# bryanlimy/tf2-cyclegan

Measured on AMD Instinct MI355X. Metric: images/sec (whole node) horse2zebra 256×256, higher is better.
Workload: dtype bf16; 1 GPU; model=cyclegan-resnet9-patchgan, global_batch=4, per_gpu_batch=4, image_size=256, parallelism=dp1

## Files before the change

cyclegan_amd/ops/_hip/bind.cpp:

```cpp
#include <torch/extension.h>

namespace cyg {
at::Tensor conv2d_fwd(at::Tensor, at::Tensor, c10::optional<at::Tensor>,
                      int64_t, int64_t, int64_t, int64_t, int64_t, bool,
                      int64_t, double);
at::Tensor convt2d_fwd(at::Tensor, at::Tensor, c10::optional<at::Tensor>,
                       int64_t, int64_t, int64_t, int64_t, int64_t, int64_t,
                       double);
std::vector<at::Tensor> conv2d_fwd_stats(at::Tensor, at::Tensor,
                                         c10::optional<at::Tensor>, int64_t,
                                         int64_t, int64_t, int64_t, int64_t,
                                         bool, int64_t, double);
std::vector<at::Tensor> convt2d_fwd_stats(at::Tensor, at::Tensor,
                                          c10::optional<at::Tensor>, int64_t,
                                          int64_t, int64_t, int64_t, int64_t,
                                          int64_t, double);
at::Tensor conv2d_dgrad(at::Tensor, at::Tensor, int64_t, int64_t, int64_t,
                        int64_t, int64_t, int64_t, int64_t, bool);
at::Tensor reflect_dgrad_rowmap(int64_t, int64_t, int64_t, int64_t, int64_t,
                                int64_t, int64_t, int64_t, int64_t, bool,
                                bool);
at::Tensor convt2d_dgrad(at::Tensor, at::Tensor, int64_t, int64_t, int64_t,
                         int64_t, int64_t);
at::Tensor conv2d_wgrad(at::Tensor, at::Tensor, int64_t, int64_t, int64_t,
// ... 23 lines not shown
                                     c10::optional<at::Tensor>, int64_t);
std::vector<at::Tensor> instnorm_fwd_q8(at::Tensor, at::Tensor, at::Tensor,
                                        double, int64_t, double,
                                        c10::optional<at::Tensor>,
                                        c10::optional<at::Tensor>,
                                        c10::optional<at::Tensor>, int64_t,
                                        at::Tensor, at::Tensor);
std::vector<at::Tensor> instnorm_bwd(at::Tensor, at::Tensor, at::Tensor,
                                     at::Tensor, at::Tensor,
                                     c10::optional<at::Tensor>, int64_t,
                                     double, c10::optional<at::Tensor>,
                                     c10::optional<at::Tensor>,
                                     c10::optional<at::Tensor>, bool);
at::Tensor act_bwd(at::Tensor, at::Tensor, int64_t, double);
at::Tensor channel_sum(at::Tensor, c10::optional<at::Tensor>, bool);
at::Tensor reflect_pad_fwd(at::Tensor, int64_t, int64_t, int64_t, int64_t);
at::Tensor reflect_pad_bwd(at::Tensor, int64_t, int64_t, int64_t, int64_t);
at::Tensor persample_loss_fwd(at::Tensor, at::Tensor, bool);
at::Tensor persample_loss_const_fwd(at::Tensor, double, bool);
std::vector<at::Tensor> persample_loss_bwd(at::Tensor, at::Tensor, at::Tensor,
                                           bool, bool, bool);
at::Tensor persample_loss_const_bwd(at::Tensor, double, at::Tensor, bool);
void adam_step_dev(at::Tensor, at::Tensor, at::Tensor, at::Tensor, at::Tensor,
                   double, double, double);
void adam_ema_step(at::Tensor, at::Tensor, at::Tensor, at::Tensor, at::Tensor,
                   double, double, double, double, int64_t, double);
void adam_ema_step_dev(at::Tensor, at::Tensor, at::Tensor, at::Tensor,
                       at::Tensor, at::Tensor, double, double, double, double);
void shadow_gather(at::Tensor, at::Tensor, at::Tensor);
void shadow_fold(at::Tensor, at::Tensor, at::Tensor);
void fold_upconv_dw_into(at::Tensor, at::Tensor, bool, bool);
void adam_step(at::Tensor, at::Tensor, at::Tensor, at::Tensor, double, double,
               double, double, int64_t);
at::Tensor augment_batch(at::Tensor, at::Tensor, at::Tensor, int64_t, int64_t,
                         at::Tensor);
at::Tensor pool_exchange(at::Tensor, at::Tensor, at::Tensor, at::Tensor);
std::vector<at::Tensor> ssim_fwd(at::Tensor, at::Tensor, int64_t);
at::Tensor ssim_bwd(at::Tensor, at::Tensor, at::Tensor, at::Tensor, at::Tensor,
                    at::Tensor);
}

PYBIND11_MODULE(TORCH_EXTENSION_NAME, m) {
  m.def("conv2d_fwd", &cyg::conv2d_fwd);
  m.def("convt2d_fwd", &cyg::convt2d_fwd);
  m.def("conv2d_fwd_stats", &cyg::conv2d_fwd_stats);
  m.def("convt2d_fwd_stats", &cyg::convt2d_fwd_stats);
  m.def("conv2d_dgrad", &cyg::conv2d_dgrad);
  m.def("reflect_dgrad_rowmap", &cyg::reflect_dgrad_rowmap, py::arg("B"),
        py::arg("H"), py::arg("W"), py::arg("pt"), py::arg("pb"),
        py::arg("pl"), py::arg("pr"), py::arg("KH"), py::arg("KW"),
        py::arg("trim") = true, py::arg("frame") = false);
  m.def("convt2d_dgrad", &cyg::convt2d_dgrad);
  m.def("conv2d_wgrad", &cyg::conv2d_wgrad);
  m.def("conv2d_wgrad_into", &cyg::conv2d_wgrad_into, py::arg("x"),
        py::arg("dy"), py::arg("kh"), py::arg("kw"), py::arg("stride"),
        py::arg("pt"), py::arg("pl"), py::arg("reflect"), py::arg("out"),
// ... 13 lines not shown
  m.def("instnorm_fwd", &cyg::instnorm_fwd, py::arg("x"), py::arg("gamma"),
        py::arg("beta"), py::arg("eps"), py::arg("act"), py::arg("slope"),
        py::arg("residual"), py::arg("psum") = py::none(),
        py::arg("psq") = py::none(), py::arg("nslabs") = 0);
  m.def("instnorm_fwd_q8", &cyg::instnorm_fwd_q8, py::arg("x"),
        py::arg("gamma"), py::arg("beta"), py::arg("eps"), py::arg("act"),
        py::arg("slope"), py::arg("residual"), py::arg("psum"),
        py::arg("psq"), py::arg("nslabs"), py::arg("amax_prev"),
        py::arg("amax_cur"));
  m.def("instnorm_bwd", &cyg::instnorm_bwd, py::arg("dy"), py::arg("x"),
        py::arg("gamma"), py::arg("mean"), py::arg("rstd"), py::arg("yact"),
        py::arg("act"), py::arg("slope"), py::arg("beta") = py::none(),
        py::arg("dgamma_out") = py::none(), py::arg("dbeta_out") = py::none(),
        py::arg("accumulate") = false);
  m.def("act_bwd", &cyg::act_bwd);
  m.def("channel_sum", &cyg::channel_sum, py::arg("x"),
        py::arg("out") = py::none(), py::arg("accumulate") = false);
  m.def("reflect_pad_fwd", &cyg::reflect_pad_fwd);
  m.def("reflect_pad_bwd", &cyg::reflect_pad_bwd);
  m.def("persample_loss_fwd", &cyg::persample_loss_fwd);
  m.def("persample_loss_const_fwd", &cyg::persample_loss_const_fwd);
  m.def("persample_loss_bwd", &cyg::persample_loss_bwd);
  m.def("persample_loss_const_bwd", &cyg::persample_loss_const_bwd);
  m.def("adam_step", &cyg::adam_step);
  m.def("adam_step_dev", &cyg::adam_step_dev);
  m.def("adam_ema_step", &cyg::adam_ema_step);
  m.def("adam_ema_step_dev", &cyg::adam_ema_step_dev);
  m.def("shadow_gather", &cyg::shadow_gather);
  m.def("shadow_fold", &cyg::shadow_fold);
  m.def("fold_upconv_dw_into", &cyg::fold_upconv_dw_into, py::arg("dv"),
        py::arg("out"), py::arg("accumulate"), py::arg("transposed"));
  m.def("augment_batch", &cyg::augment_batch);
  m.def("pool_exchange", &cyg::pool_exchange);
  m.def("ssim_fwd", &cyg::ssim_fwd, py::arg("y_true"), py::arg("y_pred"),
        py::arg("save_maps") = 0);
  m.def("ssim_bwd", &cyg::ssim_bwd, py::arg("x"), py::arg("y"), py::arg("am"),
        py::arg("bm"), py::arg("cm"), py::arg("dout"));
}
```

cyclegan_amd/ops/_hip/common.h:

```cpp
#pragma once

#include <hip/hip_runtime.h>
#include <hip/hip_bf16.h>
#include <hip/hip_fp8.h>

#define DEV __device__ __forceinline__

typedef __bf16 bf16r;
typedef bf16r v8bf __attribute__((ext_vector_type(8)));
typedef float v4f __attribute__((ext_vector_type(4)));
typedef short v8s __attribute__((ext_vector_type(8)));

DEV float b2f(short raw) {
  union { float f; unsigned u; } v;
  v.u = ((unsigned)(unsigned short)raw) << 16;
  return v.f;
}

DEV short f2b(float f) {
  __hip_bfloat16 h = __float2bfloat16(f);
  return *reinterpret_cast<short*>(&h);
}

DEV float delayed_sx(float amax_prev) {
  return fminf(448.f / fmaxf(amax_prev, 1e-12f), 65504.f);
}

DEV unsigned char f2e4m3(float f, float s) {
  __hip_fp8_e4m3 q(f * s);
  return q.__x;
}

#define ACT_NONE 0
#define ACT_RELU 1
// ... 23 lines not shown
```

cyclegan_amd/ops/_hip/norm_elem.hip:

```cpp

#include <torch/extension.h>
#include <ATen/cuda/CUDAContext.h>

#include "common.h"

namespace cyg {

constexpr int NT = 256;

static inline int cdiv64(long a, long b) { return (int)((a + b - 1) / b); }

__global__ __launch_bounds__(NT) void in_reduce_kernel(
    const short* __restrict__ x, float* __restrict__ psum,
    float* __restrict__ psq, int B, long HW, int C, int S) {
  int b = blockIdx.x / S;
  int sl = blockIdx.x % S;
  long rows = (HW + S - 1) / S;
  long r0 = sl * rows, r1 = min(r0 + rows, HW);
  const int gpr = C / 8;
  const int tid = threadIdx.x;
  const short* xb = x + (long)b * HW * C;

  int g = tid % gpr;
  int rstep = NT / gpr;
// ... 564 lines not shown
  if (i >= D) return;
  float t = use_const ? cconst : b2f(yt[base + i]);
  float p = b2f(yp[base + i]);
  float d = p - t;
  float g = dout[b] / (float)D;
  float gpv = squared ? 2.f * d * g : (d > 0.f ? g : (d < 0.f ? -g : 0.f));
  if (gp) gp[base + i] = f2b(gpv);
  if (gt) gt[base + i] = f2b(-gpv);
  (void)n;
}

__device__ __forceinline__ void adam_elem(float& p, float g, float& m,
                                          float& v, float lr_t, float b1,
                                          float b2, float eps) {
#pragma clang fp contract(off)
  float gi = g;
  float mi = b1 * m + (1.f - b1) * gi;
  float vi = b2 * v + (1.f - b2) * gi * gi;
  m = mi;
  v = vi;
  p -= lr_t * mi / (sqrtf(vi) + eps);
}

__global__ void adam_kernel(float* __restrict__ p, const float* __restrict__ g,
                            float* __restrict__ m, float* __restrict__ v,
                            long n, float lr_t, float b1, float b2,
                            float eps) {
  long i = (long)blockIdx.x * blockDim.x + threadIdx.x;
  long stride = (long)gridDim.x * blockDim.x;
  for (; i < n; i += stride)
    adam_elem(p[i], g[i], m[i], v[i], lr_t, b1, b2, eps);
}

__global__ void adam_kernel_dev(float* __restrict__ p,
                                const float* __restrict__ g,
                                float* __restrict__ m, float* __restrict__ v,
                                long n, const float* __restrict__ lr_t_ptr,
                                float b1, float b2, float eps) {
  const float lr_t = *lr_t_ptr;
  long i = (long)blockIdx.x * blockDim.x + threadIdx.x;
  long stride = (long)gridDim.x * blockDim.x;
  for (; i < n; i += stride)
    adam_elem(p[i], g[i], m[i], v[i], lr_t, b1, b2, eps);
}

__device__ __forceinline__ void adam_ema_elem(float& p, float g, float& m,
                                              float& v, float& e, float lr_t,
                                              float b1, float b2, float eps,
                                              float d, float omd) {
#pragma clang fp contract(off)
  adam_elem(p, g, m, v, lr_t, b1, b2, eps);
  e = d * e + omd * p;
}

template <bool VEC, bool LR_DEV>
__global__ void adam_ema_kernel(float* __restrict__ p,
                                const float* __restrict__ g,
                                float* __restrict__ m, float* __restrict__ v,
                                float* __restrict__ ema, long n, float lr_imm,
                                const float* __restrict__ lr_t_ptr, float b1,
                                float b2, float eps, float d, float omd) {
  const float lr_t = LR_DEV ? *lr_t_ptr : lr_imm;
  const long tid = (long)blockIdx.x * blockDim.x + threadIdx.x;
  const long stride = (long)gridDim.x * blockDim.x;
  long done = 0;
  if (VEC) {
    const long n4 = n >> 2;
    float4* p4 = reinterpret_cast<float4*>(p);
    const float4* g4 = reinterpret_cast<const float4*>(g);
    float4* m4 = reinterpret_cast<float4*>(m);
    float4* v4 = reinterpret_cast<float4*>(v);
    float4* e4 = reinterpret_cast<float4*>(ema);
    for (long i = tid; i < n4; i += stride) {
      float4 pi = p4[i], gi = g4[i], mi = m4[i], vi = v4[i], ei = e4[i];
      adam_ema_elem(pi.x, gi.x, mi.x, vi.x, ei.x, lr_t, b1, b2, eps, d, omd);
      adam_ema_elem(pi.y, gi.y, mi.y, vi.y, ei.y, lr_t, b1, b2, eps, d, omd);
      adam_ema_elem(pi.z, gi.z, mi.z, vi.z, ei.z, lr_t, b1, b2, eps, d, omd);
      adam_ema_elem(pi.w, gi.w, mi.w, vi.w, ei.w, lr_t, b1, b2, eps, d, omd);
      m4[i] = mi;
      v4[i] = vi;
      p4[i] = pi;
      e4[i] = ei;
    }
    done = n4 << 2;
  }
  for (long i = done + tid; i < n; i += stride)
    adam_ema_elem(p[i], g[i], m[i], v[i], ema[i], lr_t, b1, b2, eps, d, omd);
}


static int slices_for(long HW, int B) {
  int s = (int)std::min<long>(std::max<long>(1, 512 / std::max(B, 1)),
                              std::max<long>(1, HW / 64));
  return std::max(1, s);
}

static std::vector<at::Tensor> instnorm_fwd_impl(
    at::Tensor x, at::Tensor gamma, at::Tensor beta, double eps, int64_t act,
    double slope, c10::optional<at::Tensor> residual,
    c10::optional<at::Tensor> psum_in, c10::optional<at::Tensor> psq_in,
    int64_t nslabs, const at::Tensor* amax_prev, at::Tensor* amax_cur) {
  TORCH_CHECK(x.is_cuda() && x.scalar_type() == at::kBFloat16 && x.is_contiguous());
  int B = x.size(0), C = x.size(3);
  long HW = (long)x.size(1) * x.size(2);
  TORCH_CHECK(C % 8 == 0 && (C / 8) <= 256 && 256 % std::min(C / 8, 256) == 0,
              "instnorm: unsupported channel count ", C);
  auto stream = at::cuda::getCurrentCUDAStream();
  auto fopt = x.options().dtype(at::kFloat);
  int S = slices_for(HW, B);
  auto mean = at::empty({B, C}, fopt);
// ... 320 lines not shown
                     (const short*)yp.const_data_ptr(),
                     (const float*)dout.const_data_ptr(),
                     need_gt ? (short*)gt.mutable_data_ptr() : nullptr,
                     need_gp ? (short*)gp.mutable_data_ptr() : nullptr, D,
                     squared ? 1 : 0, 0.f, 0);
  return {gt, gp};
}

at::Tensor persample_loss_const_bwd(at::Tensor yp, double cconst,
                                    at::Tensor dout, bool squared) {
  int B = yp.size(0);
  long D = yp.numel() / B;
  auto gp = at::empty_like(yp);
  dim3 grid(cdiv64(D, 256), B);
  hipLaunchKernelGGL(persample_loss_bwd_kernel, grid, dim3(256), 0,
                     at::cuda::getCurrentCUDAStream(), nullptr,
                     (const short*)yp.const_data_ptr(),
                     (const float*)dout.const_data_ptr(), nullptr,
                     (short*)gp.mutable_data_ptr(), D, squared ? 1 : 0,
                     (float)cconst, 1);
  return gp;
}

void adam_step(at::Tensor p, at::Tensor g, at::Tensor m, at::Tensor v,
               double lr, double b1, double b2, double eps, int64_t t) {
  TORCH_CHECK(p.is_cuda() && p.scalar_type() == at::kFloat);
  long n = p.numel();
  double lr_t = lr * std::sqrt(1.0 - std::pow(b2, (double)t)) /
                (1.0 - std::pow(b1, (double)t));
  int blocks = (int)std::min<long>(2048, (n + 255) / 256);
  hipLaunchKernelGGL(adam_kernel, dim3(blocks), dim3(256), 0,
                     at::cuda::getCurrentCUDAStream(),
                     (float*)p.mutable_data_ptr(),
                     (const float*)g.const_data_ptr(),
                     (float*)m.mutable_data_ptr(),
                     (float*)v.mutable_data_ptr(), n, (float)lr_t, (float)b1,
                     (float)b2, (float)eps);
}

void adam_step_dev(at::Tensor p, at::Tensor g, at::Tensor m, at::Tensor v,
                   at::Tensor lr_t, double b1, double b2, double eps) {
  TORCH_CHECK(p.is_cuda() && p.scalar_type() == at::kFloat);
  TORCH_CHECK(lr_t.is_cuda() && lr_t.scalar_type() == at::kFloat);
  long n = p.numel();
  int blocks = (int)std::min<long>(2048, (n + 255) / 256);
  hipLaunchKernelGGL(adam_kernel_dev, dim3(blocks), dim3(256), 0,
                     at::cuda::getCurrentCUDAStream(),
                     (float*)p.mutable_data_ptr(),
                     (const float*)g.const_data_ptr(),
                     (float*)m.mutable_data_ptr(),
                     (float*)v.mutable_data_ptr(), n,
                     (const float*)lr_t.const_data_ptr(), (float)b1,
                     (float)b2, (float)eps);
}

static void adam_ema_launch(at::Tensor& p, at::Tensor& g, at::Tensor& m,
                            at::Tensor& v, at::Tensor& ema, float lr_imm,
                            const float* lr_t_ptr, double b1, double b2,
                            double eps, double ema_decay) {
  TORCH_CHECK(p.is_cuda() && p.scalar_type() == at::kFloat);
  for (const at::Tensor* t : {&p, &g, &m, &v, &ema}) {
    TORCH_CHECK(t->scalar_type() == at::kFloat, "adam_ema: fp32 only");
    TORCH_CHECK(t->numel() == p.numel(), "adam_ema: numel mismatch");
    TORCH_CHECK(t->is_contiguous(), "adam_ema: contiguous only");
    TORCH_CHECK(t->device() == p.device(), "adam_ema: device mismatch");
  }
  TORCH_CHECK(ema_decay >= 0.0 && ema_decay <= 1.0);
  long n = p.numel();
  if (n == 0) return;
  float* pp = (float*)p.mutable_data_ptr();
  const float* gp = (const float*)g.const_data_ptr();
  float* mp = (float*)m.mutable_data_ptr();
  float* vp = (float*)v.mutable_data_ptr();
  float* ep = (float*)ema.mutable_data_ptr();
  bool vec = ((reinterpret_cast<uintptr_t>(pp) |
               reinterpret_cast<uintptr_t>(gp) |
               reinterpret_cast<uintptr_t>(mp) |
               reinterpret_cast<uintptr_t>(vp) |
               reinterpret_cast<uintptr_t>(ep)) & 15) == 0;
  float d = (float)ema_decay, omd = (float)(1.0 - ema_decay);
  long work = vec ? std::max<long>(n >> 2, n & 3) : n;
  int blocks = (int)std::min<long>(2048, (work + 255) / 256);
  auto stream = at::cuda::getCurrentCUDAStream();
#define CYG_ADAM_EMA(VEC, LRD)                                              \
  hipLaunchKernelGGL((adam_ema_kernel<VEC, LRD>), dim3(blocks), dim3(256),  \
                     0, stream, pp, gp, mp, vp, ep, n, lr_imm, lr_t_ptr,    \
                     (float)b1, (float)b2, (float)eps, d, omd)
  if (lr_t_ptr) {
    if (vec) CYG_ADAM_EMA(true, true); else CYG_ADAM_EMA(false, true);
  } else {
    if (vec) CYG_ADAM_EMA(true, false); else CYG_ADAM_EMA(false, false);
  }
#undef CYG_ADAM_EMA
}

void adam_ema_step(at::Tensor p, at::Tensor g, at::Tensor m, at::Tensor v,
                   at::Tensor ema, double lr, double b1, double b2,
                   double eps, int64_t t, double ema_decay) {
  double lr_t = lr * std::sqrt(1.0 - std::pow(b2, (double)t)) /
                (1.0 - std::pow(b1, (double)t));
  adam_ema_launch(p, g, m, v, ema, (float)lr_t, nullptr, b1, b2, eps,
                  ema_decay);
}

void adam_ema_step_dev(at::Tensor p, at::Tensor g, at::Tensor m, at::Tensor v,
                       at::Tensor ema, at::Tensor lr_t, double b1, double b2,
                       double eps, double ema_decay) {
  TORCH_CHECK(lr_t.is_cuda() && lr_t.scalar_type() == at::kFloat &&
              lr_t.numel() == 1 && lr_t.device() == p.device());
  adam_ema_launch(p, g, m, v, ema, 0.f, (const float*)lr_t.const_data_ptr(),
                  b1, b2, eps, ema_decay);
}

}
```

cyclegan_amd/ops/_hip/shadow.hip:

```cpp

#include <torch/extension.h>
#include <ATen/cuda/CUDAContext.h>

#include "common.h"

namespace cyg {

constexpr int SG_NT = 256;

typedef int v8i __attribute__((ext_vector_type(8)));

__global__ __launch_bounds__(SG_NT) void shadow_gather_kernel(
    const float* __restrict__ src, const int* __restrict__ idx,
    short* __restrict__ out, long n8) {
  long t = (long)blockIdx.x * SG_NT + threadIdx.x;
  long stride = (long)gridDim.x * SG_NT;
  for (; t < n8; t += stride) {
    v8i ix = *(const v8i*)(idx + t * 8);
    v8s o;
    #pragma unroll
    for (int j = 0; j < 8; ++j)
      o[j] = ix[j] >= 0 ? f2b(src[ix[j]]) : (short)0;
    *(v8s*)(out + t * 8) = o;
  }
}

void shadow_gather(at::Tensor src, at::Tensor idx, at::Tensor out) {
  TORCH_CHECK(src.is_cuda() && src.scalar_type() == at::kFloat &&
              src.is_contiguous());
  TORCH_CHECK(idx.is_cuda() && idx.scalar_type() == at::kInt &&
              idx.is_contiguous());
  TORCH_CHECK(out.is_cuda() && out.scalar_type() == at::kBFloat16 &&
              out.is_contiguous());
  TORCH_CHECK(idx.numel() == out.numel() && idx.numel() % 8 == 0);
  long n8 = idx.numel() / 8;
  int blocks = (int)min((long)4096, (n8 + SG_NT - 1) / SG_NT);
  hipLaunchKernelGGL(shadow_gather_kernel, dim3(blocks), dim3(SG_NT), 0,
                     at::cuda::getCurrentCUDAStream(),
                     (const float*)src.const_data_ptr(),
                     (const int*)idx.const_data_ptr(),
                     (short*)out.mutable_data_ptr(), n8);
}

typedef int v4i __attribute__((ext_vector_type(4)));

__global__ __launch_bounds__(SG_NT) void shadow_fold_kernel(
    const float* __restrict__ src, const int* __restrict__ idx4,
    short* __restrict__ out, long n8) {
  long t = (long)blockIdx.x * SG_NT + threadIdx.x;
  long stride = (long)gridDim.x * SG_NT;
  for (; t < n8; t += stride) {
    v8s o;
    #pragma unroll
    for (int j = 0; j < 8; ++j) {
      v4i ix = *(const v4i*)(idx4 + (t * 8 + j) * 4);
      float s = 0.f;
      #pragma unroll
      for (int q = 0; q < 4; ++q)
        if (ix[q] >= 0) s += src[ix[q]];
      o[j] = f2b(s);
    }
    *(v8s*)(out + t * 8) = o;
  }
}
// ... 68 lines not shown
```

cyclegan_amd/ops/adam.py:

```python

from __future__ import annotations

import math

import torch

from . import backend


class FusedAdam:

    def __init__(self, flat_param: torch.Tensor, flat_grad: torch.Tensor,
                 lr: float = 2e-4, beta1: float = 0.5, beta2: float = 0.9,
                 eps: float = 1e-7, ema_decay: float = 0.0):
        assert flat_param.dtype == torch.float32
        assert 0.0 <= ema_decay < 1.0
        self.p = flat_param
        self.g = flat_grad
        self.lr, self.b1, self.b2, self.eps = lr, beta1, beta2, eps
        self.m = torch.zeros_like(flat_param)
        self.v = torch.zeros_like(flat_param)
        self.t = 0
        self.lr_scale = 1.0
        self.ema_decay = float(ema_decay)
        self.ema = flat_param.detach().clone() if ema_decay > 0 else None
        self.graph_mode = False
        self._lr_t_dev = None

    def _lr_t(self) -> float:
        return (self.lr * self.lr_scale * math.sqrt(1 - self.b2 ** self.t)
                / (1 - self.b1 ** self.t))

    @torch.no_grad()
    def reset_ema(self):
        if self.ema is not None:
            self.ema.copy_(self.p)

    @torch.no_grad()
    def prepare_graph(self):
        self.graph_mode = True
        if self._lr_t_dev is None:
            self._lr_t_dev = torch.zeros(1, dtype=torch.float32,
                                         device=self.p.device)

    @torch.no_grad()
    def advance_lr(self):
        self.t += 1
        if self._lr_t_dev is None:
            self._lr_t_dev = torch.empty(1, dtype=torch.float32,
                                         device=self.p.device)
        self._lr_t_dev.fill_(self._lr_t())

    @torch.no_grad()
    def step(self):
        if self.graph_mode:
            if self.ema is not None:
                backend.ext().adam_ema_step_dev(
                    self.p, self.g, self.m, self.v, self.ema, self._lr_t_dev,
                    self.b1, self.b2, self.eps, self.ema_decay)
                return
            backend.ext().adam_step_dev(self.p, self.g, self.m, self.v,
                                        self._lr_t_dev, self.b1, self.b2,
                                        self.eps)
            return
        self.t += 1
        if backend.use_hip(self.p):
            lr = self.lr * self.lr_scale
            if self.ema is not None:
                backend.ext().adam_ema_step(
                    self.p, self.g, self.m, self.v, self.ema, lr, self.b1,
                    self.b2, self.eps, self.t, self.ema_decay)
            else:
                backend.ext().adam_step(self.p, self.g, self.m, self.v,
                                        lr, self.b1, self.b2, self.eps, self.t)
            torch.autograd.graph.increment_version(self.p)
            return
        lr_t = (self.lr * self.lr_scale * math.sqrt(1 - self.b2 ** self.t)
                / (1 - self.b1 ** self.t))
        self.m.mul_(self.b1).add_(self.g, alpha=1 - self.b1)
        self.v.mul_(self.b2).addcmul_(self.g, self.g, value=1 - self.b2)
        self.p.addcdiv_(self.m, self.v.sqrt().add_(self.eps), value=-lr_t)
        if self.ema is not None:
            self.ema.mul_(self.ema_decay).add_(self.p, alpha=1 - self.ema_decay)

    def state_dict(self):
        return {"m": self.m, "v": self.v, "t": self.t,
                "lr": self.lr, "b1": self.b1, "b2": self.b2, "eps": self.eps}

    def load_state_dict(self, sd):
        self.m.copy_(sd["m"])
        self.v.copy_(sd["v"])
        self.t = sd["t"]
        self.lr, self.b1, self.b2, self.eps = sd["lr"], sd["b1"], sd["b2"], sd["eps"]
```

cyclegan_amd/ops/arena.py:

```python

from __future__ import annotations

from typing import Dict, List, Tuple

import torch

from . import backend

_PAD = 8


def _conv_like(m: torch.nn.Module) -> bool:
    return type(m).__name__ == "ConvNHWC"


def _convt_like(m: torch.nn.Module) -> bool:
    return type(m).__name__ == "ConvTransposeNHWC"


def _upconv_like(m: torch.nn.Module) -> bool:
    return type(m).__name__ == "UpsampleConvNHWC"


FOLD_M = ((0, 0, 1), (0, 1, 1), (1, 1, 0), (1, 0, 0))
_FOLD_TAPS = tuple(tuple(d for d in range(3) if row[d]) for row in FOLD_M)


def _idx_up(base: int, shape) -> torch.Tensor:
    O, KH, KW, I = shape
    assert KH == 3 and KW == 3
    o = torch.arange(O).view(-1, 1)
    i = torch.arange(I).view(1, -1)
# ... 54 lines not shown
    assert KW == 7
    d = torch.arange(8).view(-1, 1, 1, 1, 1, 1)
    co = torch.arange(8).view(1, -1, 1, 1, 1, 1)
    ty = torch.arange(KH).view(1, 1, -1, 1, 1, 1)
    blk = torch.arange(2).view(1, 1, 1, -1, 1, 1)
    pos = torch.arange(8).view(1, 1, 1, 1, -1, 1)
    ci = torch.arange(I).view(1, 1, 1, 1, 1, -1)
    tx = blk * 8 + pos - d
    idx = base + ((co * KH + ty) * KW + tx) * I + ci
    ok = (tx >= 0) & (tx < KW) & (co < O)
    idx = torch.where(ok, idx, torch.tensor(-1))
    return idx.reshape(64, KH, 2, 8 * I).to(torch.int32)


def _idx_packb(base: int, n: int) -> torch.Tensor:
    co = torch.arange(8).repeat(8)
    idx = base + co
    idx[co >= n] = -1
    return idx.to(torch.int32)


class ShadowArena:

    def __init__(self, group, module: torch.nn.Module):
        self.group = group
        dev = group.flat_param.device
        off = {p: o for p, (o, _) in zip(group.params, group._offsets)}

        pieces: List[torch.Tensor] = []
        plan: List[Tuple[torch.nn.Parameter, str, Tuple[int, ...], int]] = []
        total = 0
        fpieces: List[torch.Tensor] = []
        fplan: List[Tuple[torch.nn.Parameter, str, Tuple[int, ...], int]] = []
        ftotal = 0
        for m in module.modules():
            if _upconv_like(m):
                w = m.weight
                for name, fn in (("up", _idx_up), ("up_t", _idx_up_t)):
                    idx = fn(off[w], tuple(w.shape))
                    fpieces.append(idx.reshape(-1, 4))
                    fplan.append((w, name, tuple(idx.shape[:-1]), ftotal))
                    ftotal += idx.numel() // 4
                continue
            if _conv_like(m):
                forms = (("p", _idx_p), ("tp", _idx_tp))
            elif _convt_like(m):
                forms = (("plain", _idx_plain), ("t", _idx_t))
            else:
                continue
            w = m.weight
            forms = list(forms)
            packed = (_conv_like(m) and head_packable(
                tuple(w.shape), m.stride, m.pad_mode, m.padding
                if not isinstance(m.padding, str) else (0,) * 4))
            if packed:
                forms.append(("packp", _idx_packp))
            for name, fn in forms:
                idx = fn(off[w], tuple(w.shape))
                pieces.append(idx.reshape(-1))
                plan.append((w, name, tuple(idx.shape), total))
                total += idx.numel()
            if m.bias is not None:
                idx = _idx_bias(off[m.bias], m.bias.numel())
                pieces.append(idx.reshape(-1))
                plan.append((m.bias, "bias_p", tuple(idx.shape), total))
                total += idx.numel()
                if packed:
                    idx = _idx_packb(off[m.bias], m.bias.numel())
                    pieces.append(idx.reshape(-1))
                    plan.append((m.bias, "packb", tuple(idx.shape), total))
                    total += idx.numel()

        pad = (-total) % 8
        if pad:
            pieces.append(torch.full((pad,), -1, dtype=torch.int32))
        self.idx = torch.cat(pieces).to(dev) if pieces else \
            torch.empty(0, dtype=torch.int32, device=dev)
        self.buf = torch.empty(self.idx.numel(), dtype=torch.bfloat16, device=dev)

        fpad = (-ftotal) % 8
        if fpad:
            fpieces.append(torch.full((fpad, 4), -1, dtype=torch.int32))
        self.fold_idx = torch.cat(fpieces).to(dev) if fpieces else \
            torch.empty((0, 4), dtype=torch.int32, device=dev)
        self.fold_buf = torch.empty(self.fold_idx.shape[0],
                                    dtype=torch.bfloat16, device=dev)

        self.views: Dict[Tuple[int, str], torch.Tensor] = {}
        self._by_param: Dict[torch.Tensor, Dict[str, torch.Tensor]] = {}
        for p, name, shape, start in plan:
            v = self.buf[start:start + int(torch.tensor(shape).prod())].view(shape)
            self._by_param.setdefault(p, {})[name] = v
        for p, name, shape, start in fplan:
            v = self.fold_buf[start:start + int(torch.tensor(shape).prod())]
            self._by_param.setdefault(p, {})[name] = v.view(shape)

        self.refresh()

    def refresh(self):
        if self.idx.numel():
            backend.ext().shadow_gather(self.group.flat_param, self.idx, self.buf)
        if self.fold_idx.numel():
            backend.ext().shadow_fold(self.group.flat_param, self.fold_idx,
                                      self.fold_buf)

    def forms_of(self, p: torch.Tensor):
        return self._by_param.get(p)
```

cyclegan_amd/trainer.py:

```python

from __future__ import annotations

import contextlib
import os
from typing import Dict, Optional

import torch

from .models import Generator, Discriminator
from .ops import MAE, MSE, MSE_const, SSIM, ImagePool, backend, grad_sink
from .ops.adam import FusedAdam
from .parallel import DistContext, GradSync, FlatParamGroup


def lr_factor(epoch: int, epochs: int, decay_epochs: int) -> float:
    if decay_epochs <= 0:
        return 1.0
    f = 1.0 - max(0, epoch - (epochs - decay_epochs) + 1) / (decay_epochs + 1)
    return min(1.0, max(0.0, f))


class CycleGAN:
    LAMBDA_CYCLE = 10.0
    LAMBDA_IDENTITY = 0.5 * 10.0
# ... 28 lines not shown
        for m in (self.G, self.F, self.X, self.Y):
            ctx.broadcast_module(m)

        self.groups = {name: FlatParamGroup(getattr(self, name))
                       for name in self._NAMES}
        self.ema_decay = float(getattr(args, "ema_decay", 0.0) or 0.0)
        self.lr_decay_epochs = int(getattr(args, "lr_decay_epochs", 0) or 0)
        self.optimizers = {
            name: FusedAdam(g.flat_param, g.flat_grad,
                            ema_decay=self.ema_decay if name in "GF" else 0.0)
            for name, g in self.groups.items()}
        self.sync = GradSync(ctx, timing=getattr(args, "verbose", 1) == 2)

        self.arenas = {}
        if (self.device.type == "cuda"
                and self.compute_dtype == torch.bfloat16
                and backend.load_ext() is not None):
            from .ops.arena import ShadowArena
            from .ops import shadow as _shadow
            for name in self._NAMES:
                a = ShadowArena(self.groups[name], getattr(self, name))
                _shadow.register_arena(a)
                self.arenas[name] = a

        self.pool_size = int(getattr(args, "pool_size", 0) or 0)
        self._pool_seed = (int(getattr(args, "seed", 1234)), int(ctx.rank))
        self.pools = None
        self._step_codes = None
        self._static_codes = None

        self.cycle_ssim = float(getattr(args, "cycle_ssim", 0.0) or 0.0)
        if not 0.0 <= self.cycle_ssim <= 1.0:
            raise ValueError("cycle_ssim must be in [0, 1]")
        self.test_ssim = (bool(getattr(args, "test_ssim", False))
                          or self.cycle_ssim > 0.0)
        self._test_keys = self._TEST_KEYS + (
            self._SSIM_KEYS if self.test_ssim else ())

        self.graphed = None

    def _refresh_shadows(self):
        for a in self.arenas.values():
            a.refresh()

    def _snapshot_state(self):
        opts = self.optimizers
        return ({n: (g.flat_param.clone(), opts[n].m.clone(),
                     opts[n].v.clone(), opts[n].t)
                 for n, g in self.groups.items()},
                {n: o.ema.clone() for n, o in opts.items()
                 if o.ema is not None},
                [p.state_dict() for p in self.pools or ()])

    @torch.no_grad()
    def _restore_state(self, saved):
        state, emas, pools = saved
        for n, (p, m, v, t) in state.items():
            self.groups[n].flat_param.copy_(p)
            self.optimizers[n].m.copy_(m)
            self.optimizers[n].v.copy_(v)
            self.optimizers[n].t = t
        for n, e in emas.items():
            self.optimizers[n].ema.copy_(e)
        for p, s in zip(self.pools or (), pools):
            p.load_state_dict(s)
        self._refresh_shadows()
# ... 174 lines not shown

    _GROUP_LOSS = tuple(zip(_NAMES, ("loss_G/total", "loss_F/total",
                                     "loss_X/loss", "loss_Y/loss")))

    def _grads_for(self, losses: Dict[str, torch.Tensor], name: str,
                   retain: bool):
        key = dict(self._GROUP_LOSS)[name]
        group = self.groups[name]
        sink = group.grad_sink()
        with grad_sink.active(sink):
            grads = torch.autograd.grad(losses[key], group.params,
                                        retain_graph=retain,
                                        allow_unused=sink is not None)
        group.set_grads(grads, sink)

    def _retain(self, i: int) -> bool:
        return i < 3 and not self.pool_size

    def _optimize(self, roll_amax: bool = True):
        for opt in self.optimizers.values():
            opt.step()
        for g in self.groups.values():
            g.bump_versions()
        self._refresh_shadows()
        if self._fp8 and roll_amax:
            from .ops import fp8_state
            fp8_state.roll()

    def train_step(self, x, y) -> Dict[str, torch.Tensor]:
        x, y = self._cast(x), self._cast(y)
        if x.shape[0] == 0:
            return self._empty_train_step()
        if self.pool_size:
            self._step_codes = self._static_codes or tuple(
                pool.next_codes(x.shape[0])
                for pool in self._ensure_pools(x.shape[1:]))
        losses = self._forward_losses(x, y)
        for i, (name, _) in enumerate(self._GROUP_LOSS):
            self._grads_for(losses, name, retain=self._retain(i))
            self.sync.launch(self.groups[name].flat_grad)
        self.sync.wait_all()
        self._optimize()
        return {k: losses[k].detach() for k in self._TRAIN_KEYS}

    @torch.no_grad()
    def cycle_step(self, x, y, training: bool = False):
        x, y = self._cast(x), self._cast(y)
# ... 195 lines not shown
```

Baseline: 357.1 images/s.

## Write bf16 parameter mirror from Adam and serve plain/transposed weight views from it

The Adam kernels can now also write a bf16 copy of the updated fp32 parameters into a contiguous mirror buffer. Plain and padded weight forms become direct views into that mirror, and transposed forms come from a new tiled transpose kernel instead of index-based gathers. This is meant to replace the per-step gather from fp32 with streaming writes fused into the optimizer. The cost is an extra bf16 store in Adam, extra memory for the mirror and transpose buffers, and new alignment and shape conditions that decide which weights can use the mirror.

New measurement: 361.4 images/s, median of 6. 1.01x the previous value.

```diff
diff --git a/cyclegan_amd/ops/_hip/bind.cpp b/cyclegan_amd/ops/_hip/bind.cpp
--- a/cyclegan_amd/ops/_hip/bind.cpp
+++ b/cyclegan_amd/ops/_hip/bind.cpp
@@ -69,16 +69,20 @@
                                            bool, bool, bool);
 at::Tensor persample_loss_const_bwd(at::Tensor, double, at::Tensor, bool);
 void adam_step_dev(at::Tensor, at::Tensor, at::Tensor, at::Tensor, at::Tensor,
-                   double, double, double);
+                   double, double, double, c10::optional<at::Tensor>);
 void adam_ema_step(at::Tensor, at::Tensor, at::Tensor, at::Tensor, at::Tensor,
-                   double, double, double, double, int64_t, double);
+                   double, double, double, double, int64_t, double,
+                   c10::optional<at::Tensor>);
 void adam_ema_step_dev(at::Tensor, at::Tensor, at::Tensor, at::Tensor,
-                       at::Tensor, at::Tensor, double, double, double, double);
+                       at::Tensor, at::Tensor, double, double, double, double,
+                       c10::optional<at::Tensor>);
 void shadow_gather(at::Tensor, at::Tensor, at::Tensor);
+void shadow_cast(at::Tensor, at::Tensor);
+void shadow_transpose(at::Tensor, at::Tensor, at::Tensor, at::Tensor);
 void shadow_fold(at::Tensor, at::Tensor, at::Tensor);
 void fold_upconv_dw_into(at::Tensor, at::Tensor, bool, bool);
 void adam_step(at::Tensor, at::Tensor, at::Tensor, at::Tensor, double, double,
-               double, double, int64_t);
+               double, double, int64_t, c10::optional<at::Tensor>);
 at::Tensor augment_batch(at::Tensor, at::Tensor, at::Tensor, int64_t, int64_t,
                          at::Tensor);
 at::Tensor pool_exchange(at::Tensor, at::Tensor, at::Tensor, at::Tensor);
@@ -138,11 +142,25 @@
   m.def("persample_loss_const_fwd", &cyg::persample_loss_const_fwd);
   m.def("persample_loss_bwd", &cyg::persample_loss_bwd);
   m.def("persample_loss_const_bwd", &cyg::persample_loss_const_bwd);
-  m.def("adam_step", &cyg::adam_step);
-  m.def("adam_step_dev", &cyg::adam_step_dev);
-  m.def("adam_ema_step", &cyg::adam_ema_step);
-  m.def("adam_ema_step_dev", &cyg::adam_ema_step_dev);
+  m.def("adam_step", &cyg::adam_step, py::arg("p"), py::arg("g"),
+        py::arg("m"), py::arg("v"), py::arg("lr"), py::arg("b1"),
+        py::arg("b2"), py::arg("eps"), py::arg("t"),
+        py::arg("shadow") = py::none());
+  m.def("adam_step_dev", &cyg::adam_step_dev, py::arg("p"), py::arg("g"),
+        py::arg("m"), py::arg("v"), py::arg("lr_t"), py::arg("b1"),
+        py::arg("b2"), py::arg("eps"), py::arg("shadow") = py::none());
+  m.def("adam_ema_step", &cyg::adam_ema_step, py::arg("p"), py::arg("g"),
+        py::arg("m"), py::arg("v"), py::arg("ema"), py::arg("lr"),
+        py::arg("b1"), py::arg("b2"), py::arg("eps"), py::arg("t"),
+        py::arg("ema_decay"), py::arg("shadow") = py::none());
+  m.def("adam_ema_step_dev", &cyg::adam_ema_step_dev, py::arg("p"),
+        py::arg("g"), py::arg("m"), py::arg("v"), py::arg("ema"),
+        py::arg("lr_t"), py::arg("b1"), py::arg("b2"), py::arg("eps"),
+        py::arg("ema_decay"), py::arg("shadow") = py::none());
   m.def("shadow_gather", &cyg::shadow_gather);
+  m.def("shadow_cast", &cyg::shadow_cast);
+  m.def("shadow_transpose", &cyg::shadow_transpose, py::arg("src"),
+        py::arg("table"), py::arg("table_dev"), py::arg("dst"));
   m.def("shadow_fold", &cyg::shadow_fold);
   m.def("fold_upconv_dw_into", &cyg::fold_upconv_dw_into, py::arg("dv"),
         py::arg("out"), py::arg("accumulate"), py::arg("transposed"));
diff --git a/cyclegan_amd/ops/_hip/common.h b/cyclegan_amd/ops/_hip/common.h
--- a/cyclegan_amd/ops/_hip/common.h
+++ b/cyclegan_amd/ops/_hip/common.h
@@ -10,6 +10,7 @@
 typedef bf16r v8bf __attribute__((ext_vector_type(8)));
 typedef float v4f __attribute__((ext_vector_type(4)));
 typedef short v8s __attribute__((ext_vector_type(8)));
+typedef short v4s __attribute__((ext_vector_type(4)));
 
 DEV float b2f(short raw) {
   union { float f; unsigned u; } v;
diff --git a/cyclegan_amd/ops/_hip/norm_elem.hip b/cyclegan_amd/ops/_hip/norm_elem.hip
--- a/cyclegan_amd/ops/_hip/norm_elem.hip
+++ b/cyclegan_amd/ops/_hip/norm_elem.hip
@@ -610,26 +610,33 @@
   p -= lr_t * mi / (sqrtf(vi) + eps);
 }
 
+template <bool SHADOW>
 __global__ void adam_kernel(float* __restrict__ p, const float* __restrict__ g,
                             float* __restrict__ m, float* __restrict__ v,
                             long n, float lr_t, float b1, float b2,
-                            float eps) {
+                            float eps, short* __restrict__ shadow) {
   long i = (long)blockIdx.x * blockDim.x + threadIdx.x;
   long stride = (long)gridDim.x * blockDim.x;
-  for (; i < n; i += stride)
+  for (; i < n; i += stride) {
     adam_elem(p[i], g[i], m[i], v[i], lr_t, b1, b2, eps);
-}
-
+    if (SHADOW) shadow[i] = f2b(p[i]);
+  }
+}
+
+template <bool SHADOW>
 __global__ void adam_kernel_dev(float* __restrict__ p,
                                 const float* __restrict__ g,
                                 float* __restrict__ m, float* __restrict__ v,
                                 long n, const float* __restrict__ lr_t_ptr,
-                                float b1, float b2, float eps) {
+                                float b1, float b2, float eps,
+                                short* __restrict__ shadow) {
   const float lr_t = *lr_t_ptr;
   long i = (long)blockIdx.x * blockDim.x + threadIdx.x;
   long stride = (long)gridDim.x * blockDim.x;
-  for (; i < n; i += stride)
+  for (; i < n; i += stride) {
     adam_elem(p[i], g[i], m[i], v[i], lr_t, b1, b2, eps);
+    if (SHADOW) shadow[i] = f2b(p[i]);
+  }
 }
 
 __device__ __forceinline__ void adam_ema_elem(float& p, float g, float& m,
@@ -641,13 +648,14 @@
   e = d * e + omd * p;
 }
 
-template <bool VEC, bool LR_DEV>
+template <bool VEC, bool LR_DEV, bool SHADOW>
 __global__ void adam_ema_kernel(float* __restrict__ p,
                                 const float* __restrict__ g,
                                 float* __restrict__ m, float* __restrict__ v,
                                 float* __restrict__ ema, long n, float lr_imm,
                                 const float* __restrict__ lr_t_ptr, float b1,
-                                float b2, float eps, float d, float omd) {
+                                float b2, float eps, float d, float omd,
+                                short* __restrict__ shadow) {
   const float lr_t = LR_DEV ? *lr_t_ptr : lr_imm;
   const long tid = (long)blockIdx.x * blockDim.x + threadIdx.x;
   const long stride = (long)gridDim.x * blockDim.x;
@@ -669,11 +677,17 @@
       v4[i] = vi;
       p4[i] = pi;
       e4[i] = ei;
+      if (SHADOW) {
+        v4s s = {f2b(pi.x), f2b(pi.y), f2b(pi.z), f2b(pi.w)};
+        reinterpret_cast<v4s*>(shadow)[i] = s;
+      }
     }
     done = n4 << 2;
   }
-  for (long i = done + tid; i < n; i += stride)
+  for (long i = done + tid; i < n; i += stride) {
     adam_ema_elem(p[i], g[i], m[i], v[i], ema[i], lr_t, b1, b2, eps, d, omd);
+    if (SHADOW) shadow[i] = f2b(p[i]);
+  }
 }
 
 
@@ -1040,43 +1054,67 @@
   return gp;
 }
 
+static short* adam_shadow_ptr(const c10::optional<at::Tensor>& shadow,
+                              const at::Tensor& p) {
+  if (!shadow.has_value()) return nullptr;
+  const at::Tensor& s = *shadow;
+  TORCH_CHECK(s.is_cuda() && s.device() == p.device() &&
+                  s.scalar_type() == at::kBFloat16 && s.is_contiguous() &&
+                  s.numel() >= p.numel(),
+              "adam: shadow must be a contiguous bf16 tensor on the "
+              "parameters' device, at least as long as they are");
+  return (short*)s.mutable_data_ptr();
+}
+
 void adam_step(at::Tensor p, at::Tensor g, at::Tensor m, at::Tensor v,
-               double lr, double b1, double b2, double eps, int64_t t) {
+               double lr, double b1, double b2, double eps, int64_t t,
+               c10::optional<at::Tensor> shadow) {
   TORCH_CHECK(p.is_cuda() && p.scalar_type() == at::kFloat);
   long n = p.numel();
+  short* sp = adam_shadow_ptr(shadow, p);
   double lr_t = lr * std::sqrt(1.0 - std::pow(b2, (double)t)) /
                 (1.0 - std::pow(b1, (double)t));
   int blocks = (int)std::min<long>(2048, (n + 255) / 256);
-  hipLaunchKernelGGL(adam_kernel, dim3(blocks), dim3(256), 0,
-                     at::cuda::getCurrentCUDAStream(),
-                     (float*)p.mutable_data_ptr(),
-                     (const float*)g.const_data_ptr(),
-                     (float*)m.mutable_data_ptr(),
-                     (float*)v.mutable_data_ptr(), n, (float)lr_t, (float)b1,
-                     (float)b2, (float)eps);
+#define CYG_ADAM(SH)                                                        \
+  hipLaunchKernelGGL(adam_kernel<SH>, dim3(blocks), dim3(256), 0,           \
+                     at::cuda::getCurrentCUDAStream(),                      \
+                     (float*)p.mutable_data_ptr(),                          \
+                     (const float*)g.const_data_ptr(),                      \
+                     (float*)m.mutable_data_ptr(),                          \
+                     (float*)v.mutable_data_ptr(), n, (float)lr_t,          \
+                     (float)b1, (float)b2, (float)eps, sp)
+  if (sp) CYG_ADAM(true); else CYG_ADAM(false);
+#undef CYG_ADAM
 }
 
 void adam_step_dev(at::Tensor p, at::Tensor g, at::Tensor m, at::Tensor v,
-                   at::Tensor lr_t, double b1, double b2, double eps) {
+                   at::Tensor lr_t, double b1, double b2, double eps,
+                   c10::optional<at::Tensor> shadow) {
   TORCH_CHECK(p.is_cuda() && p.scalar_type() == at::kFloat);
   TORCH_CHECK(lr_t.is_cuda() && lr_t.scalar_type() == at::kFloat);
   long n = p.numel();
+  short* sp = adam_shadow_ptr(shadow, p);
   int blocks = (int)std::min<long>(2048, (n + 255) / 256);
-  hipLaunchKernelGGL(adam_kernel_dev, dim3(blocks), dim3(256), 0,
-                     at::cuda::getCurrentCUDAStream(),
-                     (float*)p.mutable_data_ptr(),
-                     (const float*)g.const_data_ptr(),
-                     (float*)m.mutable_data_ptr(),
-                     (float*)v.mutable_data_ptr(), n,
-                     (const float*)lr_t.const_data_ptr(), (float)b1,
-                     (float)b2, (float)eps);
+#define CYG_ADAM_DEV(SH)                                                    \
+  hipLaunchKernelGGL(adam_kernel_dev<SH>, dim3(blocks), dim3(256), 0,       \
+                     at::cuda::getCurrentCUDAStream(),                      \
+                     (float*)p.mutable_data_ptr(),                          \
+                     (const float*)g.const_data_ptr(),                      \
+                     (float*)m.mutable_data_ptr(),                          \
+                     (float*)v.mutable_data_ptr(), n,                       \
+                     (const float*)lr_t.const_data_ptr(), (float)b1,        \
+                     (float)b2, (float)eps, sp)
+  if (sp) CYG_ADAM_DEV(true); else CYG_ADAM_DEV(false);
+#undef CYG_ADAM_DEV
 }
 
 static void adam_ema_launch(at::Tensor& p, at::Tensor& g, at::Tensor& m,
                             at::Tensor& v, at::Tensor& ema, float lr_imm,
                             const float* lr_t_ptr, double b1, double b2,
-                            double eps, double ema_decay) {
+                            double eps, double ema_decay,
+                            const c10::optional<at::Tensor>& shadow) {
   TORCH_CHECK(p.is_cuda() && p.scalar_type() == at::kFloat);
+  short* sp = adam_shadow_ptr(shadow, p);
   for (const at::Tensor* t : {&p, &g, &m, &v, &ema}) {
     TORCH_CHECK(t->scalar_type() == at::kFloat, "adam_ema: fp32 only");
     TORCH_CHECK(t->numel() == p.numel(), "adam_ema: numel mismatch");
@@ -1095,15 +1133,25 @@
                reinterpret_cast<uintptr_t>(gp) |
                reinterpret_cast<uintptr_t>(mp) |
                reinterpret_cast<uintptr_t>(vp) |
-               reinterpret_cast<uintptr_t>(ep)) & 15) == 0;
+               reinterpret_cast<uintptr_t>(ep)) & 15) == 0 &&
+             (reinterpret_cast<uintptr_t>(sp) & 7) == 0;
   float d = (float)ema_decay, omd = (float)(1.0 - ema_decay);
   long work = vec ? std::max<long>(n >> 2, n & 3) : n;
   int blocks = (int)std::min<long>(2048, (work + 255) / 256);
   auto stream = at::cuda::getCurrentCUDAStream();
 #define CYG_ADAM_EMA(VEC, LRD)                                              \
-  hipLaunchKernelGGL((adam_ema_kernel<VEC, LRD>), dim3(blocks), dim3(256),  \
-                     0, stream, pp, gp, mp, vp, ep, n, lr_imm, lr_t_ptr,    \
-                     (float)b1, (float)b2, (float)eps, d, omd)
+  do {                                                                      \
+    if (sp)                                                                 \
+      hipLaunchKernelGGL((adam_ema_kernel<VEC, LRD, true>), dim3(blocks),   \
+                         dim3(256), 0, stream, pp, gp, mp, vp, ep, n,       \
+                         lr_imm, lr_t_ptr, (float)b1, (float)b2,            \
+                         (float)eps, d, omd, sp);                           \
+    else                                                                    \
+      hipLaunchKernelGGL((adam_ema_kernel<VEC, LRD, false>), dim3(blocks),  \
+                         dim3(256), 0, stream, pp, gp, mp, vp, ep, n,       \
+                         lr_imm, lr_t_ptr, (float)b1, (float)b2,            \
+                         (float)eps, d, omd, sp);                           \
+  } while (0)
   if (lr_t_ptr) {
     if (vec) CYG_ADAM_EMA(true, true); else CYG_ADAM_EMA(false, true);
   } else {
@@ -1114,20 +1162,22 @@
 
 void adam_ema_step(at::Tensor p, at::Tensor g, at::Tensor m, at::Tensor v,
                    at::Tensor ema, double lr, double b1, double b2,
-                   double eps, int64_t t, double ema_decay) {
+                   double eps, int64_t t, double ema_decay,
+                   c10::optional<at::Tensor> shadow) {
   double lr_t = lr * std::sqrt(1.0 - std::pow(b2, (double)t)) /
                 (1.0 - std::pow(b1, (double)t));
   adam_ema_launch(p, g, m, v, ema, (float)lr_t, nullptr, b1, b2, eps,
-                  ema_decay);
+                  ema_decay, shadow);
 }
 
 void adam_ema_step_dev(at::Tensor p, at::Tensor g, at::Tensor m, at::Tensor v,
                        at::Tensor ema, at::Tensor lr_t, double b1, double b2,
-                       double eps, double ema_decay) {
+                       double eps, double ema_decay,
+                       c10::optional<at::Tensor> shadow) {
   TORCH_CHECK(lr_t.is_cuda() && lr_t.scalar_type() == at::kFloat &&
               lr_t.numel() == 1 && lr_t.device() == p.device());
   adam_ema_launch(p, g, m, v, ema, 0.f, (const float*)lr_t.const_data_ptr(),
-                  b1, b2, eps, ema_decay);
-}
-
-}
+                  b1, b2, eps, ema_decay, shadow);
+}
+
+}
diff --git a/cyclegan_amd/ops/_hip/shadow.hip b/cyclegan_amd/ops/_hip/shadow.hip
--- a/cyclegan_amd/ops/_hip/shadow.hip
+++ b/cyclegan_amd/ops/_hip/shadow.hip
@@ -40,6 +40,131 @@
                      (const float*)src.const_data_ptr(),
                      (const int*)idx.const_data_ptr(),
                      (short*)out.mutable_data_ptr(), n8);
+}
+
+__global__ __launch_bounds__(SG_NT) void shadow_cast_kernel(
+    const float* __restrict__ src, short* __restrict__ out, long n) {
+  const long tid = (long)blockIdx.x * SG_NT + threadIdx.x;
+  const long stride = (long)gridDim.x * SG_NT;
+  const long n8 = n >> 3;
+  for (long t = tid; t < n8; t += stride) {
+    v4f a = *(const v4f*)(src + t * 8);
+    v4f b = *(const v4f*)(src + t * 8 + 4);
+    v8s o = {f2b(a[0]), f2b(a[1]), f2b(a[2]), f2b(a[3]),
+             f2b(b[0]), f2b(b[1]), f2b(b[2]), f2b(b[3])};
+    *(v8s*)(out + t * 8) = o;
+  }
+  for (long i = (n8 << 3) + tid; i < n; i += stride) out[i] = f2b(src[i]);
+}
+
+void shadow_cast(at::Tensor src, at::Tensor out) {
+  TORCH_CHECK(src.is_cuda() && src.scalar_type() == at::kFloat &&
+              src.is_contiguous());
+  TORCH_CHECK(out.is_cuda() && out.scalar_type() == at::kBFloat16 &&
+              out.is_contiguous() && out.device() == src.device());
+  TORCH_CHECK(out.numel() >= src.numel(), "shadow_cast: out too short");
+  TORCH_CHECK(((reinterpret_cast<uintptr_t>(src.const_data_ptr()) |
+                reinterpret_cast<uintptr_t>(out.const_data_ptr())) & 15) == 0,
+              "shadow_cast: 16-byte aligned buffers only");
+  long n = src.numel();
+  if (n == 0) return;
+  long work = std::max<long>(n >> 3, n & 7);
+  int blocks = (int)min((long)4096, (work + SG_NT - 1) / SG_NT);
+  hipLaunchKernelGGL(shadow_cast_kernel, dim3(blocks), dim3(SG_NT), 0,
+                     at::cuda::getCurrentCUDAStream(),
+                     (const float*)src.const_data_ptr(),
+                     (short*)out.mutable_data_ptr(), n);
+}
+
+constexpr int ST_COLS = 8;
+constexpr int ST_T = 64;
+constexpr int ST_LD = ST_T + 8;
+
+__global__ __launch_bounds__(SG_NT) void shadow_transpose_kernel(
+    const short* __restrict__ src, const int* __restrict__ table, int rows,
+    short* __restrict__ dst) {
+  __shared__ __attribute__((aligned(16))) short tile[ST_T * ST_LD];
+  const int blk = blockIdx.x;
+  int r = 0;
+  while (r + 1 < rows && table[(r + 1) * ST_COLS + 5] <= blk) ++r;
+  const int* row = table + r * ST_COLS;
+  const long src_off = row[0], dst_off = row[1];
+  const int Cout = row[2], taps = row[3], Cin = row[4];
+  const int tci = row[6], tco = row[7];
+  int local = blk - row[5];
+  const int ci0 = (local % tci) * ST_T;
+  local /= tci;
+  const int co0 = (local % tco) * ST_T;
+  const int tap = local / tco;
+  if (tap >= taps) return;
+
+  #pragma unroll
+  for (int k = 0; k < (ST_T * ST_T / 8) / SG_NT; ++k) {
+    const int w = threadIdx.x + k * SG_NT;
+    const int co = co0 + w / (ST_T / 8);
+    const int cw = (w % (ST_T / 8)) * 8;
+    if (co < Cout && ci0 + cw < Cin) {
+      v8s x = *(const v8s*)(src + src_off +
+                            ((long)co * taps + tap) * Cin + ci0 + cw);
+      #pragma unroll
+      for (int j = 0; j < 8; ++j) tile[(cw + j) * ST_LD + (co - co0)] = x[j];
+    }
+  }
+  __syncthreads();
+  #pragma unroll
+  for (int k = 0; k < (ST_T * ST_T / 8) / SG_NT; ++k) {
+    const int w = threadIdx.x + k * SG_NT;
+    const int ci = ci0 + w / (ST_T / 8);
+    const int cw = (w % (ST_T / 8)) * 8;
+    if (ci < Cin && co0 + cw < Cout) {
+      v8s x = *(const v8s*)(tile + (ci - ci0) * ST_LD + cw);
+      *(v8s*)(dst + dst_off + ((long)ci * taps + tap) * Cout + co0 + cw) = x;
+    }
+  }
+}
+
+void shadow_transpose(at::Tensor src, at::Tensor table, at::Tensor table_dev,
+                      at::Tensor dst) {
+  TORCH_CHECK(src.is_cuda() && src.scalar_type() == at::kBFloat16 &&
+              src.is_contiguous());
+  TORCH_CHECK(dst.is_cuda() && dst.scalar_type() == at::kBFloat16 &&
+              dst.is_contiguous() && dst.device() == src.device());
+  TORCH_CHECK(!table.is_cuda() && table.scalar_type() == at::kInt &&
+              table.is_contiguous() && table.dim() == 2 &&
+              table.size(1) == ST_COLS);
+  TORCH_CHECK(table_dev.is_cuda() && table_dev.device() == src.device() &&
+              table_dev.scalar_type() == at::kInt &&
+              table_dev.is_contiguous() &&
+              table_dev.sizes() == table.sizes());
+  TORCH_CHECK(((reinterpret_cast<uintptr_t>(src.const_data_ptr()) |
+                reinterpret_cast<uintptr_t>(dst.const_data_ptr())) & 15) == 0,
+              "shadow_transpose: 16-byte aligned buffers only");
+  const int rows = (int)table.size(0);
+  if (rows == 0) return;
+  const int* t = (const int*)table.const_data_ptr();
+  long blocks = 0;
+  for (int r = 0; r < rows; ++r) {
+    const int* row = t + r * ST_COLS;
+    const long so = row[0], d_o = row[1], Cout = row[2], taps = row[3],
+               Cin = row[4];
+    TORCH_CHECK(Cout > 0 && taps > 0 && Cin > 0 && Cout % 8 == 0 &&
+                    Cin % 8 == 0 && so >= 0 && d_o >= 0 && so % 8 == 0 &&
+                    d_o % 8 == 0,
+                "shadow_transpose: row ", r, " is not eligible");
+    const long n = Cout * taps * Cin;
+    TORCH_CHECK(so + n <= src.numel() && d_o + n <= dst.numel(),
+                "shadow_transpose: row ", r, " out of bounds");
+    const long tci = (Cin + ST_T - 1) / ST_T, tco = (Cout + ST_T - 1) / ST_T;
+    TORCH_CHECK(row[5] == blocks && row[6] == tci && row[7] == tco,
+                "shadow_transpose: row ", r, " has a wrong block layout");
+    blocks += taps * tci * tco;
+  }
+  TORCH_CHECK(blocks < (1L << 31));
+  hipLaunchKernelGGL(shadow_transpose_kernel, dim3((unsigned)blocks),
+                     dim3(SG_NT), 0, at::cuda::getCurrentCUDAStream(),
+                     (const short*)src.const_data_ptr(),
+                     (const int*)table_dev.const_data_ptr(), rows,
+                     (short*)dst.mutable_data_ptr());
 }
 
 typedef int v4i __attribute__((ext_vector_type(4)));
diff --git a/cyclegan_amd/ops/adam.py b/cyclegan_amd/ops/adam.py
--- a/cyclegan_amd/ops/adam.py
+++ b/cyclegan_amd/ops/adam.py
@@ -26,6 +26,8 @@
         self.ema = flat_param.detach().clone() if ema_decay > 0 else None
         self.graph_mode = False
         self._lr_t_dev = None
+        self.shadow = None
+        self.wrote_shadow = False
 
     def _lr_t(self) -> float:
         return (self.lr * self.lr_scale * math.sqrt(1 - self.b2 ** self.t)
@@ -53,26 +55,30 @@
 
     @torch.no_grad()
     def step(self):
+        self.wrote_shadow = False
         if self.graph_mode:
+            self.wrote_shadow = self.shadow is not None
             if self.ema is not None:
                 backend.ext().adam_ema_step_dev(
                     self.p, self.g, self.m, self.v, self.ema, self._lr_t_dev,
-                    self.b1, self.b2, self.eps, self.ema_decay)
+                    self.b1, self.b2, self.eps, self.ema_decay, self.shadow)
                 return
             backend.ext().adam_step_dev(self.p, self.g, self.m, self.v,
                                         self._lr_t_dev, self.b1, self.b2,
-                                        self.eps)
+                                        self.eps, self.shadow)
             return
         self.t += 1
         if backend.use_hip(self.p):
             lr = self.lr * self.lr_scale
+            self.wrote_shadow = self.shadow is not None
             if self.ema is not None:
                 backend.ext().adam_ema_step(
                     self.p, self.g, self.m, self.v, self.ema, lr, self.b1,
-                    self.b2, self.eps, self.t, self.ema_decay)
+                    self.b2, self.eps, self.t, self.ema_decay, self.shadow)
             else:
                 backend.ext().adam_step(self.p, self.g, self.m, self.v,
-                                        lr, self.b1, self.b2, self.eps, self.t)
+                                        lr, self.b1, self.b2, self.eps, self.t,
+                                        self.shadow)
             torch.autograd.graph.increment_version(self.p)
             return
         lr_t = (self.lr * self.lr_scale * math.sqrt(1 - self.b2 ** self.t)
diff --git a/cyclegan_amd/ops/arena.py b/cyclegan_amd/ops/arena.py
--- a/cyclegan_amd/ops/arena.py
+++ b/cyclegan_amd/ops/arena.py
@@ -1,13 +1,37 @@
 
 from __future__ import annotations
 
-from typing import Dict, List, Tuple
+import os
+from typing import Dict, List, Optional, Tuple
 
 import torch
 
 from . import backend
 
 _PAD = 8
+
+_ST_COLS = 8
+_ST_T = 64
+
+
+def mirror_enabled() -> bool:
+    return os.environ.get("CYG_NO_ADAM_SHADOW") != "1"
+
+
+def mirror_view_ok(base: int, shape) -> bool:
+    O, _, _, I = shape
+    return O >= _PAD and I >= _PAD and base % 8 == 0
+
+
+def transpose_ok(base: int, shape) -> bool:
+    O, _, _, I = shape
+    return O % 8 == 0 and I % 8 == 0 and base % 8 == 0
+
+
+def transpose_row(src: int, dst: int, shape, first_block: int) -> List[int]:
+    O, KH, KW, I = shape
+    tci, tco = -(-I // _ST_T), -(-O // _ST_T)
+    return [src, dst, O, KH * KW, I, first_block, tci, tco]
 
 
 def _conv_like(m: torch.nn.Module) -> bool:
@@ -108,9 +132,12 @@
 
 class ShadowArena:
 
-    def __init__(self, group, module: torch.nn.Module):
+    def __init__(self, group, module: torch.nn.Module,
+                 mirror: Optional[bool] = None):
         self.group = group
         dev = group.flat_param.device
+        if mirror is None:
+            mirror = group.flat_param.is_cuda and mirror_enabled()
         off = {p: o for p, (o, _) in zip(group.params, group._offsets)}
 
         pieces: List[torch.Tensor] = []
@@ -119,6 +146,10 @@
         fpieces: List[torch.Tensor] = []
         fplan: List[Tuple[torch.nn.Parameter, str, Tuple[int, ...], int]] = []
         ftotal = 0
+        vplan: List[Tuple[torch.nn.Parameter, str, Tuple[int, ...], int]] = []
+        tplan: List[Tuple[torch.nn.Parameter, str, Tuple[int, ...], int]] = []
+        trows: List[List[int]] = []
+        ttotal = tblocks = 0
         for m in module.modules():
             if _upconv_like(m):
                 w = m.weight
@@ -141,8 +172,22 @@
                 if not isinstance(m.padding, str) else (0,) * 4))
             if packed:
                 forms.append(("packp", _idx_packp))
+            shape = tuple(w.shape)
+            O, KH, KW, I = shape
             for name, fn in forms:
-                idx = fn(off[w], tuple(w.shape))
+                if mirror and name in ("p", "plain") \
+                        and mirror_view_ok(off[w], shape):
+                    vplan.append((w, name, shape, off[w]))
+                    continue
+                if mirror and name in ("tp", "t") \
+                        and transpose_ok(off[w], shape):
+                    row = transpose_row(off[w], ttotal, shape, tblocks)
+                    trows.append(row)
+                    tplan.append((w, name, (I, KH, KW, O), ttotal))
+                    ttotal += w.numel()
+                    tblocks += row[3] * row[6] * row[7]
+                    continue
+                idx = fn(off[w], shape)
                 pieces.append(idx.reshape(-1))
                 plan.append((w, name, tuple(idx.shape), total))
                 total += idx.numel()
@@ -172,23 +217,43 @@
         self.fold_buf = torch.empty(self.fold_idx.shape[0],
                                     dtype=torch.bfloat16, device=dev)
 
+        self.mirror = None
+        if mirror:
+            n = group.flat_param.numel()
+            self.mirror = torch.zeros(n + (-n) % 8, dtype=torch.bfloat16,
+                                      device=dev)
+        self.tbuf = torch.empty(ttotal, dtype=torch.bfloat16, device=dev)
+        self.ttable = torch.tensor(trows, dtype=torch.int32).reshape(
+            -1, _ST_COLS)
+        self.ttable_dev = self.ttable.to(dev)
+
         self.views: Dict[Tuple[int, str], torch.Tensor] = {}
         self._by_param: Dict[torch.Tensor, Dict[str, torch.Tensor]] = {}
-        for p, name, shape, start in plan:
-            v = self.buf[start:start + int(torch.tensor(shape).prod())].view(shape)
-            self._by_param.setdefault(p, {})[name] = v
-        for p, name, shape, start in fplan:
-            v = self.fold_buf[start:start + int(torch.tensor(shape).prod())]
-            self._by_param.setdefault(p, {})[name] = v.view(shape)
+        self.source: Dict[torch.Tensor, Dict[str, str]] = {}
+        for kind, store, entries in (("gather", self.buf, plan),
+                                     ("fold", self.fold_buf, fplan),
+                                     ("mirror", self.mirror, vplan),
+                                     ("transpose", self.tbuf, tplan)):
+            for p, name, shape, start in entries:
+                v = store[start:start + int(torch.tensor(shape).prod())]
+                self._by_param.setdefault(p, {})[name] = v.view(shape)
+                self.source.setdefault(p, {})[name] = kind
 
         self.refresh()
 
-    def refresh(self):
+    def refresh(self, mirror_fresh: bool = False):
+        ext = backend.ext()
+        if self.mirror is not None:
+            if not mirror_fresh:
+                ext.shadow_cast(self.group.flat_param, self.mirror)
+            if self.ttable.shape[0]:
+                ext.shadow_transpose(self.mirror, self.ttable,
+                                     self.ttable_dev, self.tbuf)
         if self.idx.numel():
-            backend.ext().shadow_gather(self.group.flat_param, self.idx, self.buf)
+            ext.shadow_gather(self.group.flat_param, self.idx, self.buf)
         if self.fold_idx.numel():
-            backend.ext().shadow_fold(self.group.flat_param, self.fold_idx,
-                                      self.fold_buf)
+            ext.shadow_fold(self.group.flat_param, self.fold_idx,
+                            self.fold_buf)
 
     def forms_of(self, p: torch.Tensor):
         return self._by_param.get(p)
diff --git a/cyclegan_amd/trainer.py b/cyclegan_amd/trainer.py
--- a/cyclegan_amd/trainer.py
+++ b/cyclegan_amd/trainer.py
@@ -74,6 +74,7 @@
                 a = ShadowArena(self.groups[name], getattr(self, name))
                 _shadow.register_arena(a)
                 self.arenas[name] = a
+                self.optimizers[name].shadow = a.mirror
 
         self.pool_size = int(getattr(args, "pool_size", 0) or 0)
         self._pool_seed = (int(getattr(args, "seed", 1234)), int(ctx.rank))
@@ -91,9 +92,10 @@
 
         self.graphed = None
 
-    def _refresh_shadows(self):
-        for a in self.arenas.values():
-            a.refresh()
+    def _refresh_shadows(self, after_adam: bool = False):
+        for name, a in self.arenas.items():
+            a.refresh(mirror_fresh=after_adam
+                      and self.optimizers[name].wrote_shadow)
 
     def _snapshot_state(self):
         opts = self.optimizers
@@ -314,7 +316,7 @@
             opt.step()
         for g in self.groups.values():
             g.bump_versions()
-        self._refresh_shadows()
+        self._refresh_shadows(after_adam=True)
         if self._fp8 and roll_amax:
             from .ops import fp8_state
             fp8_state.roll()
```
